# fcogidi/X3D-tf

Measured on AMD Instinct MI355X. Metric: clips/sec (fwd+bwd) X3D-M 16x224^2; depthwise HBM GB/s, higher is better.
Workload: dtype bf16

## Files before the change

### x3d-tf_amd/csrc/dw_mx.hip

```cpp
#include "dw_common.h"

#define MX_PITCH 48
#define MX_ROWS 18
#define MX_TILE (MX_PITCH * MX_ROWS)

struct DwMxFwdArgs {
  DwFwdArgs f;
  unsigned bytes;
};

template <typename T> struct MxOp;
template <> struct MxOp<bf16> {
  typedef bf16x8 x8;
  static __device__ __forceinline__ f32x4 mfma(x8 a, x8 b, f32x4 c) { return __builtin_amdgcn_mfma_f32_16x16x32_bf16(a, b, c, 0, 0, 0); }
};
template <> struct MxOp<f16> {
  typedef f16x8 x8;
  static __device__ __forceinline__ f32x4 mfma(x8 a, x8 b, f32x4 c) { return __builtin_amdgcn_mfma_f32_16x16x32_f16(a, b, c, 0, 0, 0); }
};

template <typename T, bool FLIP>
__device__ __forceinline__ void mx_weight_operands(const float* __restrict__ wc, int lane, typename MxOp<T>::x8 (&A)[6]) {
  const int w = lane & 15, g = lane >> 4;
  float wr[27];
#pragma unroll
  for (int k = 0; k < 27; k++) wr[k] = wc[k];
#pragma unroll
  for (int i = 0; i < 6; i++) {
    const int kt = i >> 1;
    float t3[3];
#pragma unroll
    for (int kw = 0; kw < 3; kw++) {
      float lo, hi;
      if (!FLIP) {
        lo = (i & 1) ? wr[kt * 9 + 6 + kw] : wr[kt * 9 + kw];
        hi = (i & 1) ? 0.f : wr[kt * 9 + 3 + kw];
      } else {
        lo = (i & 1) ? wr[(2 - kt) * 9 + 0 + (2 - kw)] : wr[(2 - kt) * 9 + 6 + (2 - kw)];
        hi = (i & 1) ? 0.f : wr[(2 - kt) * 9 + 3 + (2 - kw)];
      }
      t3[kw] = (g >> 1) ? hi : lo;
    }
    typename MxOp<T>::x8 a;
#pragma unroll
    for (int j = 0; j < 8; j++) {
      const int kw = 8 * (g & 1) + j - w + 1;
      const float v = kw == 0 ? t3[0] : (kw == 1 ? t3[1] : (kw == 2 ? t3[2] : 0.f));
      a[j] = (T)v;
    }
    A[i] = a;
  }
}

template <bool P7>
struct MxMap {
  int voffL, shift;
  int vst0, vst1, vst1e;
  unsigned mk0, mk1;
  int n;
  int planeB;
  __device__ __forceinline__ void build(int lane, int blk, int N, int C, int T, int H, int W, int& c) {
    const int h = lane & 15, s = lane >> 4;
    if constexpr (!P7) {
      c = __builtin_amdgcn_readfirstlane(blk % C);
      n = __builtin_amdgcn_readfirstlane(blk / C);
      const bool ok0 = h < H && 4 * s < W, ok1 = h < H && 4 * s + 2 < W;
      const long long e = (((long long)n * C + c) * T * H + h) * W + 4 * s;
      voffL = ok0 ? (int)(e * 2) : DW_OOB;
      shift = 0;
      vst0 = voffL;
      vst1 = ok1 ? (int)(e * 2) + 4 : DW_OOB;
      vst1e = DW_OOB;
      mk0 = ok0 ? 0xffffffffu : 0u;
      mk1 = ok1 ? 0xffffffffu : 0u;
      planeB = H * W * 2;
    } else {
      c = __builtin_amdgcn_readfirstlane(blk % C);
      const int n0 = __builtin_amdgcn_readfirstlane(blk / C) * 4;
      n = n0 + 2 * (h >> 3) + (s >> 1);
      const int r = h & 7, second = s & 1;
      const bool ok = r < 7 && n < N;
      const long long e = (((long long)n * C + c) * T * 7 + r) * 7 + 4 * second;
      voffL = ok ? (int)((e - second) * 2) : DW_OOB;
      shift = second;
      vst0 = ok ? (int)(e * 2) : DW_OOB;
      vst1 = (ok && !second) ? (int)(e * 2) + 4 : DW_OOB;
      vst1e = (ok && second) ? (int)(e * 2) + 4 : DW_OOB;
      mk0 = ok ? 0xffffffffu : 0u;
      mk1 = ok ? (second ? 0x0000ffffu : 0xffffffffu) : 0u;
      planeB = 49 * 2;
    }
  }
  __device__ __forceinline__ Raw aligned(const Raw& r) const {
    if constexpr (P7) {
      const unsigned long long v = (((unsigned long long)r.w[1] << 32) | r.w[0]) >> (16 * shift);
      Raw o; o.w[0] = (unsigned)v; o.w[1] = (unsigned)(v >> 32); o.w[2] = o.w[3] = 0u;
      return o;
    } else {
      return r;
    }
  }
  __device__ __forceinline__ void store(__amdgpu_buffer_rsrc_t rs, unsigned p0, unsigned p1, int soff) const {
    Raw o, o1;
    o.w[0] = p0; o1.w[0] = p1;
    raw_bstore<4>(o, rs, vst0, soff);
    raw_bstore<4>(o1, rs, vst1, soff);
    if constexpr (P7) raw_bstore<2>(o1, rs, vst1e, soff);
  }
};

template <typename T, int UN, int RB, int PD, bool EXACT, bool P7>
__global__ __launch_bounds__(64, 7) void dw3d_fwd_mx14_kernel(const DwMxFwdArgs pa) {
  static_assert(UN % RB == 0 && UN % PD == 0, "ring period RB, slots period PD");
  typedef typename MxOp<T>::x8 x8;
  __shared__ __attribute__((aligned(16))) unsigned char lds[RB * MX_TILE];
  const DwFwdArgs& a = pa.f;
  const DwGeom& g = a.g;
  const int lane = threadIdx.x;
  const int h = lane & 15, s = lane >> 4;
  int c;
  MxMap<P7> mp;
  mp.build(lane, blockIdx.x, g.N, g.C, g.T, g.H, g.W, c);

  for (int i = lane; i < RB * MX_TILE / 16; i += 64) ((uint4*)lds)[i] = make_uint4(0u, 0u, 0u, 0u);

  x8 A[6];
  mx_weight_operands<T, false>(a.w + c * 27, lane, A);
  float sc = 1.f, sh = 0.f;
  if (a.ss) { sc = a.ss[c * 2]; sh = a.ss[c * 2 + 1]; }
  const float lo = a.act == X3D_ACT_RELU ? 0.f : -__builtin_inff();

  const int planeB = mp.planeB;
  const __amdgpu_buffer_rsrc_t rsX = __builtin_amdgcn_make_buffer_rsrc((T*)a.x, 0, pa.bytes, 0x00020000);
  const __amdgpu_buffer_rsrc_t rsY = __builtin_amdgcn_make_buffer_rsrc((T*)a.y, 0, pa.bytes, 0x00020000);
  unsigned char* stg = lds + (h + 1) * MX_PITCH + s * 8;
  const unsigned char* rd01 = lds + (h + (s >> 1)) * MX_PITCH + (s & 1) * 16;
  const unsigned char* rd2 = lds + (h + 2) * MX_PITCH + (s & 1) * 16;

  Raw slot[PD];
  auto issue = [&](int t, Raw& r) { raw_bload<8>(r, rsX, mp.voffL, t < g.T ? t * planeB : DW_OOB); };
  const unsigned mk0 = mp.mk0, mk1 = mp.mk1;
  auto stage = [&](const Raw& r0, int q, bool plane_ok) {
    const Raw r = mp.aligned(r0);
    float v[4];
#pragma unroll
    for (int e = 0; e < 4; e++) v[e] = fmaxf(__builtin_fmaf(sc, raw_get<T>(r, e), sh), lo);
    const unsigned pm = plane_ok ? 0xffffffffu : 0u;
    *(uint2*)(stg + q * MX_TILE) = make_uint2(Dot2<T>::pk(v[0], v[1]) & (mk0 & pm), Dot2<T>::pk(v[2], v[3]) & (mk1 & pm));
  };
  float s1 = 0.f, s2 = 0.f;

  auto dummy_stores = [&]() { mp.store(rsY, 0u, 0u, DW_OOB); };
#pragma unroll
  for (int p = 0; p < PD; p++) { issue(p, slot[p]); dummy_stores(); }
  stage(slot[0], 1, true);
  issue(PD, slot[0]);
  dummy_stores();

  for (int t0 = 0; t0 < g.T; t0 += UN) {
#pragma unroll
    for (int d = 0; d < UN; d++) {
      const int t = t0 + d;
      if (!EXACT && t >= g.T) break;
      const int qm = d % RB, q0 = (d + 1) % RB, qp = (d + 2) % RB;
      stage(slot[(d + 1) % PD], qp, t + 1 < g.T);
      issue(t + 1 + PD, slot[(d + 1) % PD]);
      f32x4 acc = {0.f, 0.f, 0.f, 0.f}, acc2 = {0.f, 0.f, 0.f, 0.f};
      const int qs[3] = {qm, q0, qp};
#pragma unroll
      for (int kt = 0; kt < 3; kt++) {
        const x8 b01 = *(const x8*)(rd01 + qs[kt] * MX_TILE);
        const x8 b2 = *(const x8*)(rd2 + qs[kt] * MX_TILE);
        acc = MxOp<T>::mfma(A[2 * kt], b01, acc);
        acc2 = MxOp<T>::mfma(A[2 * kt + 1], b2, acc2);
      }
      acc += acc2;
      float o4[4];
#pragma unroll
      for (int e = 0; e < 4; e++) {
        const unsigned m = e < 2 ? mk0 : mk1;
        o4[e] = (m >> (16 * (e & 1)) & 1u) ? acc[e] : 0.f;
        s1 += o4[e];
        s2 += o4[e] * o4[e];
      }
      mp.store(rsY, Dot2<T>::pk(o4[0], o4[1]), Dot2<T>::pk(o4[2], o4[3]), t * planeB);
    }
  }
  if (a.stats || a.pool) {
    const float q1 = wave_sum(s1), q2 = wave_sum(s2);
    float qp[P7 ? 4 : 1];
    if constexpr (P7) {
#pragma unroll
      for (int k = 0; k < 4; k++) qp[k] = wave_sum((2 * (h >> 3) + (s >> 1)) == k ? s1 : 0.f);
    }
    if (lane == 0) {
      if (a.stats) {
        double* sp = stats_replica(a.stats, g.C, (unsigned)blockIdx.x);
        atomic_add_d(&sp[c * 2], (double)q1);
        atomic_add_d(&sp[c * 2 + 1], (double)q2);
      }
      if (a.pool) {
        if constexpr (P7) {
          const int n0 = (int)(blockIdx.x / g.C) * 4;
#pragma unroll
          for (int k = 0; k < 4; k++) if (n0 + k < g.N) atomic_add_d(&a.pool[(long long)(n0 + k) * g.C + c], (double)qp[k]);
        } else {
          atomic_add_d(&a.pool[(long long)mp.n * g.C + c], (double)q1);
        }
      }
    }
  }
}

static bool mx_plane_ok(const DwGeom& g, bool* p7) {
  *p7 = g.H == 7 && g.W == 7;
  return *p7 || (g.H >= 12 && g.H <= 14 && g.W >= 12 && g.W <= 14 && (g.W & 1) == 0);
}

bool dw_fwd_mx_launch(const DwFwdArgs& a, int dtype, int S, hipStream_t st) {
  const DwGeom& g = a.g;
  const int e = x3d_env_int("X3D_DW_MX", 1);
  bool p7;
  if (e == 0 || dtype == X3D_F32 || S != 1 || !mx_plane_ok(g, &p7) || a.bn.stats) return false;
  const long long bytes = (long long)g.N * g.C * g.T * g.H * g.W * 2;
  if (bytes >= (1ll << 30) || (long long)g.C * g.N >= (1ll << 31)) return false;
  if (((uintptr_t)a.x & 3) || ((uintptr_t)a.y & 3)) return false;
  const bool exact = g.T % 4 == 0;
  if (x3d_describe.out) {
    snprintf(x3d_describe.out, x3d_describe.cap, "dw3d_fwd_mx14_kernel<%s, %s, %d>", dtype == X3D_BF16 ? "bf16" : "f16",
             exact ? "4, 4, 4, 1" : "6, 3, 3, 0", (int)p7);
    return true;
  }
  DwMxFwdArgs pa;
  pa.f = a;
  pa.bytes = (unsigned)bytes;
  const dim3 grid((unsigned)(g.C * (p7 ? ceil_div(g.N, 4) : g.N)));
#define MX_FWD(TT, P7_)                                                                                             \
  do {                                                                                                              \
    if (exact) hipLaunchKernelGGL((dw3d_fwd_mx14_kernel<TT, 4, 4, 4, true, P7_>), grid, dim3(64), 0, st, pa);       \
    else hipLaunchKernelGGL((dw3d_fwd_mx14_kernel<TT, 6, 3, 3, false, P7_>), grid, dim3(64), 0, st, pa);            \
  } while (0)
  if (dtype == X3D_BF16) { if (p7) MX_FWD(bf16, true); else MX_FWD(bf16, false); }
  else { if (p7) MX_FWD(f16, true); else MX_FWD(f16, false); }
#undef MX_FWD
  return true;
}

#define MXA_PITCH 80
#define MXA_TILE (MXA_PITCH * MX_ROWS)

struct DwMxBwdArgs {
  DwBwdArgs b;
  unsigned bytes;
};

template <typename T, int UN, int RB, int PD, bool EXACT, bool P7>
__global__ __launch_bounds__(64, 3) void dw3d_bwd_mx14_kernel(const DwMxBwdArgs pa) {
  static_assert(UN % RB == 0 && UN % 2 == 0 && UN % PD == 0, "ring periods RB (dB planes), 2 (A planes) and PD (planes in flight)");
  typedef typename MxOp<T>::x8 x8;
  typedef __attribute__((ext_vector_type(4))) unsigned int u32x4_;
  __shared__ __attribute__((aligned(16))) unsigned char lds[RB * MX_TILE + 2 * MXA_TILE + 64];
  unsigned char* ldsA = lds + RB * MX_TILE;
  const DwBwdArgs& a = pa.b;
  const DwGeom& g = a.g;
  const int lane = threadIdx.x;
  const int h = lane & 15, s = lane >> 4;
  int c;
  MxMap<P7> mp;
  mp.build(lane, blockIdx.x, g.N, g.C, g.T, g.H, g.W, c);

  for (int i = lane; i < (RB * MX_TILE + 2 * MXA_TILE + 64) / 16; i += 64) ((uint4*)lds)[i] = make_uint4(0u, 0u, 0u, 0u);

  x8 Wt[6];
  mx_weight_operands<T, true>(a.w + c * 27, lane, Wt);
  const float sc = a.ss_a[c * 2], sh = a.ss_a[c * 2 + 1];
  float cA = 0.f, cB = 0.f, cC = 0.f;
  if (mp.n < g.N) {
    const float* cf = a.coef_nc + ((long long)mp.n * g.C + c) * 4;
    cA = cf[0]; cB = cf[1]; cC = cf[2];
  }
  const int planeB = mp.planeB;
  const __amdgpu_buffer_rsrc_t rsA = __builtin_amdgcn_make_buffer_rsrc((T*)a.araw, 0, pa.bytes, 0x00020000);
  const __amdgpu_buffer_rsrc_t rsD = __builtin_amdgcn_make_buffer_rsrc((T*)a.dv, 0, pa.bytes, 0x00020000);
  const __amdgpu_buffer_rsrc_t rsR = __builtin_amdgcn_make_buffer_rsrc((T*)a.braw, 0, pa.bytes, 0x00020000);
  const __amdgpu_buffer_rsrc_t rsG = __builtin_amdgcn_make_buffer_rsrc((T*)a.ga, 0, pa.bytes, 0x00020000);
  unsigned char* stgB = lds + (h + 1) * MX_PITCH + s * 8;
  const unsigned char* rd01 = lds + (h + (s >> 1)) * MX_PITCH + (s & 1) * 16;
  const unsigned char* rd2 = lds + (h + 2) * MX_PITCH + (s & 1) * 16;
  const bool lowk = s < 2;
  const unsigned char* rdM = lowk ? lds + (h + 1) * MX_PITCH + (s & 1) * 16 : lds + RB * MX_TILE + 2 * MXA_TILE;
  const int rdM_tile = lowk ? MX_TILE : 0;
  unsigned char* stgA = ldsA + (h + 1) * MXA_PITCH + 16 + s * 8;
  const unsigned char* rdN = ldsA + (h + 1) * MXA_PITCH + 16 + (s & 1) * 16;

  struct Slot { Raw A, D, R; };
  Slot slot[PD];
  auto issue = [&](int t, Slot& q) {
    const int soff = t < g.T ? t * planeB : DW_OOB;
    raw_bload<8>(q.A, rsA, mp.voffL, soff);
    raw_bload<8>(q.D, rsD, mp.voffL, soff);
    raw_bload<8>(q.R, rsR, mp.voffL, soff);
  };
  const unsigned mk0 = mp.mk0, mk1 = mp.mk1;
  auto stage = [&](const Slot& q, int qb, int qa, bool plane_ok) {
    const Raw rA = mp.aligned(q.A), rD = mp.aligned(q.D), rR = mp.aligned(q.R);
    float av[4], bv[4];
#pragma unroll
    for (int e = 0; e < 4; e++) {
      av[e] = fmaxf(__builtin_fmaf(sc, raw_get<T>(rA, e), sh), 0.f);
      bv[e] = __builtin_fmaf(cA, raw_get<T>(rD, e), __builtin_fmaf(cB, raw_get<T>(rR, e), cC));
    }
    const unsigned pm = plane_ok ? 0xffffffffu : 0u;
    const unsigned m0 = mk0 & pm, m1 = mk1 & pm;
    *(uint2*)(stgA + qa * MXA_TILE) = make_uint2(Dot2<T>::pk(av[0], av[1]) & m0, Dot2<T>::pk(av[2], av[3]) & m1);
    *(uint2*)(stgB + qb * MX_TILE) = make_uint2(Dot2<T>::pk(bv[0], bv[1]) & m0, Dot2<T>::pk(bv[2], bv[3]) & m1);
  };

  f32x4 Cw[9];
#pragma unroll
  for (int k = 0; k < 9; k++) Cw[k] = (f32x4){0.f, 0.f, 0.f, 0.f};
  float s1 = 0.f, s2 = 0.f;
  Raw own;

  auto dummy_stores = [&]() { mp.store(rsG, 0u, 0u, DW_OOB); };
#pragma unroll
  for (int p = 0; p < PD; p++) { issue(p, slot[p]); dummy_stores(); }
  stage(slot[0], 1, 0, true);
  own = mp.aligned(slot[0].A);
  issue(PD, slot[0]);
  dummy_stores();

  for (int t0 = 0; t0 < g.T; t0 += UN) {
#pragma unroll
    for (int d = 0; d < UN; d++) {
      const int t = t0 + d;
      if (!EXACT && t >= g.T) break;
      const int qs[3] = {d % RB, (d + 1) % RB, (d + 2) % RB};
      const int sl = (d + 1) % PD;
      stage(slot[sl], qs[2], (d + 1) & 1, t + 1 < g.T);
      const Raw own_next = mp.aligned(slot[sl].A);
      issue(t + 1 + PD, slot[sl]);
      f32x4 acc = {0.f, 0.f, 0.f, 0.f}, acc2 = {0.f, 0.f, 0.f, 0.f};
#pragma unroll
      for (int kt = 0; kt < 3; kt++) {
        const x8 b01 = *(const x8*)(rd01 + qs[kt] * MX_TILE);
        const x8 b2 = *(const x8*)(rd2 + qs[kt] * MX_TILE);
        acc = MxOp<T>::mfma(Wt[2 * kt], b01, acc);
        acc2 = MxOp<T>::mfma(Wt[2 * kt + 1], b2, acc2);
      }
      {
        const unsigned char* pn = rdN + (d & 1) * MXA_TILE;
        const u32x4_ mid = *(const u32x4_*)pn;
        const unsigned prv = *(const unsigned*)(pn - 4), nxt = *(const unsigned*)(pn + 16);
        const unsigned m01 = __builtin_amdgcn_alignbit(mid[1], mid[0], 16), m12 = __builtin_amdgcn_alignbit(mid[2], mid[1], 16),
                       m23 = __builtin_amdgcn_alignbit(mid[3], mid[2], 16);
        const u32x4_ lft = {__builtin_amdgcn_alignbit(mid[0], prv, 16), m01, m12, m23};
        const u32x4_ rgt = {m01, m12, m23, __builtin_amdgcn_alignbit(nxt, mid[3], 16)};
        const x8 n0 = __builtin_bit_cast(x8, lft), n1 = __builtin_bit_cast(x8, mid), n2 = __builtin_bit_cast(x8, rgt);
#pragma unroll
        for (int kt = 0; kt < 3; kt++) {
          const x8 m = *(const x8*)(rdM + qs[2 - kt] * rdM_tile);
          Cw[kt * 3 + 0] = MxOp<T>::mfma(m, n0, Cw[kt * 3 + 0]);
          Cw[kt * 3 + 1] = MxOp<T>::mfma(m, n1, Cw[kt * 3 + 1]);
          Cw[kt * 3 + 2] = MxOp<T>::mfma(m, n2, Cw[kt * 3 + 2]);
          }
      }
      acc += acc2;
      float o4[4];
#pragma unroll
      for (int e = 0; e < 4; e++) {
        const float av = raw_get<T>(own, e);
        o4[e] = (__builtin_fmaf(sc, av, sh) > 0.f && ((e < 2 ? mk0 : mk1) >> (16 * (e & 1)) & 1u)) ? acc[e] : 0.f;
        s1 += o4[e];
        s2 += o4[e] * av;
      }
      mp.store(rsG, Dot2<T>::pk(o4[0], o4[1]), Dot2<T>::pk(o4[2], o4[3]), t * planeB);
      own = own_next;
    }
  }

  float red[29];
#pragma unroll
  for (int kt = 0; kt < 3; kt++)
#pragma unroll
    for (int kw = 0; kw < 3; kw++) {
      float p[3] = {0.f, 0.f, 0.f};
#pragma unroll
      for (int r = 0; r < 4; r++) {
        const int kh = h - (4 * s + r) + 1;
        const float v = Cw[kt * 3 + kw][r];
        p[0] += kh == 0 ? v : 0.f;
        p[1] += kh == 1 ? v : 0.f;
        p[2] += kh == 2 ? v : 0.f;
      }
#pragma unroll
      for (int kh = 0; kh < 3; kh++) red[kt * 9 + kh * 3 + kw] = wave_sum_lane63(p[kh]);
    }
  red[27] = wave_sum_lane63(s1);
  red[28] = wave_sum_lane63(s2);
  dw_flush_sums29(red, lane, a.dw + c * 27, a.a_sums + c * 2);
}

bool dw_bwd_mx_launch(const DwBwdArgs& a, int dtype, int S, hipStream_t st) {
  const DwGeom& g = a.g;
  const int e = x3d_env_int("X3D_DW_MX", 1);
  bool p7;
  if (e == 0 || (dtype != X3D_BF16 && (dtype != X3D_F16 || x3d_env_int("X3D_DW_MX_F16", 1) == 0)) || S != 1 || !mx_plane_ok(g, &p7)) return false;
  if (p7 && e != 7) return false;
  const long long bytes = (long long)g.N * g.C * g.T * g.H * g.W * 2;
  if (bytes >= (1ll << 30) || (long long)g.C * g.N >= (1ll << 31)) return false;
  if (((uintptr_t)a.araw & 3) || ((uintptr_t)a.ga & 3) || ((uintptr_t)a.dv & 3) || ((uintptr_t)a.braw & 3)) return false;
  const bool exact = g.T % 4 == 0 && !(p7 && dtype != X3D_BF16);
  if (x3d_describe.out) {
    snprintf(x3d_describe.out, x3d_describe.cap, "dw3d_bwd_mx14_kernel<%s, %s, %d>", dtype == X3D_BF16 ? "bf16" : "f16", exact ? "4, 4, 2, 1" : "6, 3, 3, 0", (int)p7);
    return true;
  }
  DwMxBwdArgs pa;
  pa.b = a;
  pa.bytes = (unsigned)bytes;
  const dim3 grid((unsigned)(g.C * (p7 ? ceil_div(g.N, 4) : g.N)));
#define MX14_BWD(T_)                                                                                              \
  do {                                                                                                            \
    if (p7) {                                                                                                     \
      if (exact) hipLaunchKernelGGL((dw3d_bwd_mx14_kernel<T_, 4, 4, 2, true, true>), grid, dim3(64), 0, st, pa);    \
      else hipLaunchKernelGGL((dw3d_bwd_mx14_kernel<T_, 6, 3, 3, false, true>), grid, dim3(64), 0, st, pa);         \
    } else {                                                                                                      \
      if (exact) hipLaunchKernelGGL((dw3d_bwd_mx14_kernel<T_, 4, 4, 2, true, false>), grid, dim3(64), 0, st, pa);   \
      else hipLaunchKernelGGL((dw3d_bwd_mx14_kernel<T_, 6, 3, 3, false, false>), grid, dim3(64), 0, st, pa);        \
    }                                                                                                             \
  } while (0)
  if (dtype == X3D_BF16) MX14_BWD(bf16); else MX14_BWD(f16);
#undef MX14_BWD
  return true;
}


#define MXW_PITCH 112
#define MXW_TILE (MXW_PITCH * MX_ROWS)

struct DwMxwBwdArgs {
  DwBwdArgs b;
  unsigned bytes;
  int HT;
};

template <typename T, int UN, int RB, int PD, bool EXACT>
__global__ __launch_bounds__(64, 2) void dw3d_bwd_mxw_kernel(const DwMxwBwdArgs pa) {
  static_assert(UN % RB == 0 && UN % 2 == 0 && UN % PD == 0, "ring periods RB (dB planes), 2 (A planes) and PD (planes in flight)");
  typedef typename MxOp<T>::x8 x8;
  typedef __attribute__((ext_vector_type(4))) unsigned int u32x4_;
  __shared__ __attribute__((aligned(16))) unsigned char lds[(RB + 2) * MXW_TILE + 128];
  unsigned char* ldsA = lds + RB * MXW_TILE;
  const DwBwdArgs& a = pa.b;
  const DwGeom& g = a.g;
  const int lane = threadIdx.x;
  const int n16 = lane & 15, s = lane >> 4;
  const int ht = __builtin_amdgcn_readfirstlane(blockIdx.x % pa.HT);
  const int nc = __builtin_amdgcn_readfirstlane(blockIdx.x / pa.HT);
  const int c = nc % g.C, n = nc / g.C;
  const int H = g.H, W = g.W;
  const int r0 = ht * 14;

  for (int i = lane; i < ((RB + 2) * MXW_TILE + 128) / 16; i += 64) ((uint4*)lds)[i] = make_uint4(0u, 0u, 0u, 0u);

  x8 Wt[9];
  {
    const float* wc = a.w + c * 27;
#pragma unroll
    for (int i = 0; i < 9; i++) {
      const int kt = i / 3, kh = i % 3;
      const float* w3 = wc + (2 - kt) * 9 + (2 - kh) * 3;
      const float w0 = w3[2], w1 = w3[1], w2 = w3[0];
      x8 op;
#pragma unroll
      for (int j = 0; j < 8; j++) {
        const int kw = 8 * s + j - n16 - 7;
        op[j] = (T)(kw == 0 ? w0 : (kw == 1 ? w1 : (kw == 2 ? w2 : 0.f)));
      }
      Wt[i] = op;
    }
  }
  const float sc = a.ss_a[c * 2], sh = a.ss_a[c * 2 + 1];
  const float* cf = a.coef_nc + ((long long)n * g.C + c) * 4;
  const float cA = cf[0], cB = cf[1], cC = cf[2];

  const int planeB = H * W * 2;
  const __amdgpu_buffer_rsrc_t rsA = __builtin_amdgcn_make_buffer_rsrc((T*)a.araw, 0, pa.bytes, 0x00020000);
  const __amdgpu_buffer_rsrc_t rsD = __builtin_amdgcn_make_buffer_rsrc((T*)a.dv, 0, pa.bytes, 0x00020000);
  const __amdgpu_buffer_rsrc_t rsR = __builtin_amdgcn_make_buffer_rsrc((T*)a.braw, 0, pa.bytes, 0x00020000);
  const __amdgpu_buffer_rsrc_t rsG = __builtin_amdgcn_make_buffer_rsrc((T*)a.ga, 0, pa.bytes, 0x00020000);
  const int row = r0 - 1 + n16;
  const bool row_in = row >= 0 && row < H;
  const bool row_own = n16 >= 1 && n16 <= 14 && row < H;
  const long long base = ((long long)n * g.C + c) * g.T * H * W + (long long)row * W;
  int vld[2], vs0[2], vs1[2];
  unsigned mk0[2], mk1[2], eo0[2], eo1[2];
#pragma unroll
  for (int j = 0; j < 2; j++) {
    const int col = 16 * j + 4 * s;
    const bool c0 = col < W, c1 = col + 2 < W;
    vld[j] = (row_in && c0) ? (int)((base + col) * 2) : DW_OOB;
    mk0[j] = (row_in && c0) ? 0xffffffffu : 0u;
    mk1[j] = (row_in && c1) ? 0xffffffffu : 0u;
    eo0[j] = (row_own && c0) ? 1u : 0u;
    eo1[j] = (row_own && c1) ? 1u : 0u;
    vs0[j] = eo0[j] ? (int)((base + col) * 2) : DW_OOB;
    vs1[j] = eo1[j] ? (int)((base + col + 2) * 2) : DW_OOB;
  }
  unsigned char* stgB = lds + (n16 + 1) * MXW_PITCH + 16 + s * 8;
  unsigned char* stgA = ldsA + (n16 + 1) * MXW_PITCH + 16 + s * 8;
  const unsigned char* rdB = lds + n16 * MXW_PITCH + s * 16;
  const unsigned char* rdM = row_own ? lds + (n16 + 1) * MXW_PITCH + 16 + s * 16 : lds + (RB + 2) * MXW_TILE;
  const int rdM_tile = row_own ? MXW_TILE : 0;
  const unsigned char* rdN = ldsA + (n16 + 1) * MXW_PITCH + 16 + s * 16;

  struct Slot { Raw A[2], D[2], R[2]; };
  Slot slot[PD];
  auto issue = [&](int t, Slot& q) {
    const int soff = t < g.T ? t * planeB : DW_OOB;
#pragma unroll
    for (int j = 0; j < 2; j++) {
      raw_bload<8>(q.A[j], rsA, vld[j], soff);
      raw_bload<8>(q.D[j], rsD, vld[j], soff);
      raw_bload<8>(q.R[j], rsR, vld[j], soff);
    }
  };
  auto stage = [&](const Slot& q, int qb, int qa, bool plane_ok) {
    const unsigned pm = plane_ok ? 0xffffffffu : 0u;
#pragma unroll
    for (int j = 0; j < 2; j++) {
      float av[4], bv[4];
#pragma unroll
      for (int e = 0; e < 4; e++) {
        av[e] = fmaxf(__builtin_fmaf(sc, raw_get<T>(q.A[j], e), sh), 0.f);
        bv[e] = __builtin_fmaf(cA, raw_get<T>(q.D[j], e), __builtin_fmaf(cB, raw_get<T>(q.R[j], e), cC));
      }
      const unsigned m0 = mk0[j] & pm, m1 = mk1[j] & pm;
      *(uint2*)(stgA + qa * MXW_TILE + 32 * j) = make_uint2(Dot2<T>::pk(av[0], av[1]) & m0, Dot2<T>::pk(av[2], av[3]) & m1);
      *(uint2*)(stgB + qb * MXW_TILE + 32 * j) = make_uint2(Dot2<T>::pk(bv[0], bv[1]) & m0, Dot2<T>::pk(bv[2], bv[3]) & m1);
    }
  };
  auto store4 = [&](int j, unsigned p0, unsigned p1, int soff) {
    Raw o, o1;
    o.w[0] = p0; o1.w[0] = p1;
    raw_bstore<4>(o, rsG, vs0[j], soff);
    raw_bstore<4>(o1, rsG, vs1[j], soff);
  };
  auto dummy_stores = [&]() { store4(0, 0u, 0u, DW_OOB); store4(1, 0u, 0u, DW_OOB); };

  f32x4 Cw[9];
#pragma unroll
  for (int k = 0; k < 9; k++) Cw[k] = (f32x4){0.f, 0.f, 0.f, 0.f};
  float s1 = 0.f, s2 = 0.f;
  Raw own[2];

#pragma unroll
  for (int p = 0; p < PD; p++) { issue(p, slot[p]); dummy_stores(); }
  stage(slot[0], 1, 0, true);
  own[0] = slot[0].A[0]; own[1] = slot[0].A[1];
  issue(PD, slot[0]);
  dummy_stores();

  for (int t0 = 0; t0 < g.T; t0 += UN) {
#pragma unroll
    for (int d = 0; d < UN; d++) {
      const int t = t0 + d;
      if (!EXACT && t >= g.T) break;
      const int qs[3] = {d % RB, (d + 1) % RB, (d + 2) % RB};
      const int sl = (d + 1) % PD;
      stage(slot[sl], qs[2], (d + 1) & 1, t + 1 < g.T);
      const Raw on0 = slot[sl].A[0], on1 = slot[sl].A[1];
      issue(t + 1 + PD, slot[sl]);
      {
        const unsigned char* pn = rdN + (d & 1) * MXW_TILE;
        const u32x4_ mid = *(const u32x4_*)pn;
        const unsigned prv = *(const unsigned*)(pn - 4), nxt = *(const unsigned*)(pn + 16);
        const unsigned m01 = __builtin_amdgcn_alignbit(mid[1], mid[0], 16), m12 = __builtin_amdgcn_alignbit(mid[2], mid[1], 16),
                       m23 = __builtin_amdgcn_alignbit(mid[3], mid[2], 16);
        const u32x4_ lft = {__builtin_amdgcn_alignbit(mid[0], prv, 16), m01, m12, m23};
        const u32x4_ rgt = {m01, m12, m23, __builtin_amdgcn_alignbit(nxt, mid[3], 16)};
        const x8 n0 = __builtin_bit_cast(x8, lft), n1 = __builtin_bit_cast(x8, mid), n2 = __builtin_bit_cast(x8, rgt);
#pragma unroll
        for (int kt = 0; kt < 3; kt++) {
          const x8 m = *(const x8*)(rdM + qs[2 - kt] * rdM_tile);
          Cw[kt * 3 + 0] = MxOp<T>::mfma(m, n0, Cw[kt * 3 + 0]);
          Cw[kt * 3 + 1] = MxOp<T>::mfma(m, n1, Cw[kt * 3 + 1]);
          Cw[kt * 3 + 2] = MxOp<T>::mfma(m, n2, Cw[kt * 3 + 2]);
        }
      }
#pragma unroll
      for (int j = 0; j < 2; j++) {
        f32x4 acc = {0.f, 0.f, 0.f, 0.f}, acc2 = {0.f, 0.f, 0.f, 0.f}, acc3 = {0.f, 0.f, 0.f, 0.f};
#pragma unroll
        for (int kt = 0; kt < 3; kt++) {
          const unsigned char* pb = rdB + qs[kt] * MXW_TILE + 32 * j;
          acc = MxOp<T>::mfma(Wt[kt * 3 + 0], *(const x8*)(pb), acc);
          acc2 = MxOp<T>::mfma(Wt[kt * 3 + 1], *(const x8*)(pb + MXW_PITCH), acc2);
          acc3 = MxOp<T>::mfma(Wt[kt * 3 + 2], *(const x8*)(pb + 2 * MXW_PITCH), acc3);
        }
        acc += acc2 + acc3;
        float o4[4];
#pragma unroll
        for (int e = 0; e < 4; e++) {
          const float av = raw_get<T>(own[j], e);
          o4[e] = (__builtin_fmaf(sc, av, sh) > 0.f && (e < 2 ? eo0[j] : eo1[j])) ? acc[e] : 0.f;
          s1 += o4[e];
          s2 += o4[e] * av;
        }
        store4(j, Dot2<T>::pk(o4[0], o4[1]), Dot2<T>::pk(o4[2], o4[3]), t * planeB);
      }
      own[0] = on0; own[1] = on1;
    }
  }

  float red[29];
#pragma unroll
  for (int kt = 0; kt < 3; kt++)
#pragma unroll
    for (int kw = 0; kw < 3; kw++) {
      float p[3] = {0.f, 0.f, 0.f};
#pragma unroll
      for (int r = 0; r < 4; r++) {
        const int kh = n16 - (4 * s + r) + 1;
        const float v = Cw[kt * 3 + kw][r];
        p[0] += kh == 0 ? v : 0.f;
        p[1] += kh == 1 ? v : 0.f;
        p[2] += kh == 2 ? v : 0.f;
      }
#pragma unroll
      for (int kh = 0; kh < 3; kh++) red[kt * 9 + kh * 3 + kw] = wave_sum_lane63(p[kh]);
    }
  red[27] = wave_sum_lane63(s1);
  red[28] = wave_sum_lane63(s2);
  dw_flush_sums29(red, lane, a.dw + c * 27, a.a_sums + c * 2);
}

bool dw_bwd_mxw_launch(const DwBwdArgs& a, int dtype, int S, hipStream_t st) {
  const DwGeom& g = a.g;
  const int e = x3d_env_int("X3D_DW_MXW", 1);
  if (e == 0 || (dtype != X3D_BF16 && (dtype != X3D_F16 || x3d_env_int("X3D_DW_MX_F16", 1) == 0)) || S != 1 || (g.W & 1) || g.W < 26 || g.W > 30 || g.H < 12 ||
      (g.H % 14 != 0 && g.H % 14 < 10)) return false;
  const long long bytes = (long long)g.N * g.C * g.T * g.H * g.W * 2;
  const int HT = ceil_div(g.H, 14);
  if (bytes >= (1ll << 30) || (long long)g.C * g.N * HT >= (1ll << 31)) return false;
  if (((uintptr_t)a.araw & 7) || ((uintptr_t)a.ga & 3) || ((uintptr_t)a.dv & 7) || ((uintptr_t)a.braw & 7)) return false;
  const bool exact = g.T % 4 == 0 && dtype == X3D_BF16;
  if (x3d_describe.out) {
    snprintf(x3d_describe.out, x3d_describe.cap, "dw3d_bwd_mxw_kernel<%s, %s>", dtype == X3D_BF16 ? "bf16" : "f16", exact ? "4, 4, 2, 1" : "6, 3, 3, 0");
    return true;
  }
  DwMxwBwdArgs pa;
  pa.b = a;
  pa.bytes = (unsigned)bytes;
  pa.HT = HT;
  const dim3 grid((unsigned)((long long)g.C * g.N * HT));
  if (dtype == X3D_BF16) {
    if (exact) hipLaunchKernelGGL((dw3d_bwd_mxw_kernel<bf16, 4, 4, 2, true>), grid, dim3(64), 0, st, pa);
    else hipLaunchKernelGGL((dw3d_bwd_mxw_kernel<bf16, 6, 3, 3, false>), grid, dim3(64), 0, st, pa);
  } else {
    if (exact) hipLaunchKernelGGL((dw3d_bwd_mxw_kernel<f16, 4, 4, 2, true>), grid, dim3(64), 0, st, pa);
    else hipLaunchKernelGGL((dw3d_bwd_mxw_kernel<f16, 6, 3, 3, false>), grid, dim3(64), 0, st, pa);
  }
  return true;
}
```

Measured before the change: 3198.

## Process multiple batch samples per wave in depthwise weight-grad kernel with cross-sample streaming

The backward depthwise MFMA kernel now assigns several batch samples of the same channel and row tile to one wave, instead of one sample per wave. Weight-gradient accumulators stay in registers across samples, so each wave does one reduction and flush for all of them. In the exact path the load pipeline runs straight into the next sample, and that sample's first plane is staged early, which avoids draining and refilling the prefetch at sample boundaries. The number of samples per wave is cut back when the grid would otherwise be too small to fill the device. This adds per-sample coefficient selection and extra double-precision atomics for the activation sums, and it reduces parallelism.

```diff
diff --git a/x3d-tf_amd/csrc/dw_mx.hip b/x3d-tf_amd/csrc/dw_mx.hip
--- a/x3d-tf_amd/csrc/dw_mx.hip
+++ b/x3d-tf_amd/csrc/dw_mx.hip
@@ -442,11 +442,32 @@
   DwBwdArgs b;
   unsigned bytes;
   int HT;
+  int k;
 };
+
+#define MXW_SAMPLES 2
+#define MX_SAMPLES_MAX 4
+static int mx_samples_per_wave(int k, long long waves, int waves_per_simd) {
+  const int e = x3d_env_int("X3D_DW_MX_K", 0);
+  if (e > 0) return e < MX_SAMPLES_MAX ? e : MX_SAMPLES_MAX;
+  const long long slots = (long long)x3d_device_cus() * 4 * waves_per_simd;
+  while (k > 1 && waves / k < 2 * slots) k >>= 1;
+  return k;
+}
+
+__device__ __forceinline__ float mx_pick(const float (&kc)[MX_SAMPLES_MAX][3], int j, int e) {
+  float v = kc[MX_SAMPLES_MAX - 1][e];
+#pragma unroll
+  for (int q = MX_SAMPLES_MAX - 2; q >= 0; q--) v = j == q ? kc[q][e] : v;
+  return v;
+}
 
 template <typename T, int UN, int RB, int PD, bool EXACT>
 __global__ __launch_bounds__(64, 2) void dw3d_bwd_mxw_kernel(const DwMxwBwdArgs pa) {
   static_assert(UN % RB == 0 && UN % 2 == 0 && UN % PD == 0, "ring periods RB (dB planes), 2 (A planes) and PD (planes in flight)");
+  constexpr bool STREAM = EXACT;
+  static_assert(!STREAM || (RB == 4 && UN == 4 && PD < 4), "the stream parks the next sample's plane 0 in the ring's fourth slot; "
+                                                           "it looks PD planes into the next sample (T >= 4)");
   typedef typename MxOp<T>::x8 x8;
   typedef __attribute__((ext_vector_type(4))) unsigned int u32x4_;
   __shared__ __attribute__((aligned(16))) unsigned char lds[(RB + 2) * MXW_TILE + 128];
@@ -456,8 +477,10 @@
   const int lane = threadIdx.x;
   const int n16 = lane & 15, s = lane >> 4;
   const int ht = __builtin_amdgcn_readfirstlane(blockIdx.x % pa.HT);
-  const int nc = __builtin_amdgcn_readfirstlane(blockIdx.x / pa.HT);
-  const int c = nc % g.C, n = nc / g.C;
+  const int c = __builtin_amdgcn_readfirstlane(blockIdx.x / pa.HT);
+  const int n = (int)(blockIdx.y + blockIdx.z * 65535u) * pa.k;
+  if (n >= g.N) return;
+  const int ns = min(pa.k, g.N - n);
   const int H = g.H, W = g.W;
   const int r0 = ht * 14;
 
@@ -482,9 +505,22 @@
   }
   const float sc = a.ss_a[c * 2], sh = a.ss_a[c * 2 + 1];
   const float* cf = a.coef_nc + ((long long)n * g.C + c) * 4;
-  const float cA = cf[0], cB = cf[1], cC = cf[2];
+  float cA = cf[0], cB = cf[1], cC = cf[2];
+  float kc[MX_SAMPLES_MAX][3];
+#pragma unroll
+  for (int j = 0; j < MX_SAMPLES_MAX; j++) {
+    const float* cn = a.coef_nc + ((long long)(n + min(j, ns - 1)) * g.C + c) * 4;
+    kc[j][0] = cn[0]; kc[j][1] = cn[1]; kc[j][2] = cn[2];
+  }
+  float nA, nB, nC;
+  auto next_coef = [&](int i) { nA = mx_pick(kc, i + 1, 0); nB = mx_pick(kc, i + 1, 1); nC = mx_pick(kc, i + 1, 2); };
+  next_coef(0);
 
   const int planeB = H * W * 2;
+  const int sampB = g.C * g.T * planeB;
+  int sb = 0;
+  bool more = STREAM && ns > 1;
+  int pastB = more ? sampB - g.T * planeB : DW_OOB, pastM = more ? planeB : 0;
   const __amdgpu_buffer_rsrc_t rsA = __builtin_amdgcn_make_buffer_rsrc((T*)a.araw, 0, pa.bytes, 0x00020000);
   const __amdgpu_buffer_rsrc_t rsD = __builtin_amdgcn_make_buffer_rsrc((T*)a.dv, 0, pa.bytes, 0x00020000);
   const __amdgpu_buffer_rsrc_t rsR = __builtin_amdgcn_make_buffer_rsrc((T*)a.braw, 0, pa.bytes, 0x00020000);
@@ -517,7 +553,8 @@
   struct Slot { Raw A[2], D[2], R[2]; };
   Slot slot[PD];
   auto issue = [&](int t, Slot& q) {
-    const int soff = t < g.T ? t * planeB : DW_OOB;
+    const bool in = t < g.T;
+    const int soff = (in ? sb : pastB) + t * (in ? planeB : pastM);
 #pragma unroll
     for (int j = 0; j < 2; j++) {
       raw_bload<8>(q.A[j], rsA, vld[j], soff);
@@ -525,7 +562,7 @@
       raw_bload<8>(q.R[j], rsR, vld[j], soff);
     }
   };
-  auto stage = [&](const Slot& q, int qb, int qa, bool plane_ok) {
+  auto stage = [&](const Slot& q, int qb, int qa, bool plane_ok, bool NEXT0 = false, int qn = 0) {
     const unsigned pm = plane_ok ? 0xffffffffu : 0u;
 #pragma unroll
     for (int j = 0; j < 2; j++) {
@@ -536,8 +573,15 @@
         bv[e] = __builtin_fmaf(cA, raw_get<T>(q.D[j], e), __builtin_fmaf(cB, raw_get<T>(q.R[j], e), cC));
       }
       const unsigned m0 = mk0[j] & pm, m1 = mk1[j] & pm;
-      *(uint2*)(stgA + qa * MXW_TILE + 32 * j) = make_uint2(Dot2<T>::pk(av[0], av[1]) & m0, Dot2<T>::pk(av[2], av[3]) & m1);
+      const unsigned a0 = NEXT0 ? mk0[j] : m0, a1 = NEXT0 ? mk1[j] : m1;
+      *(uint2*)(stgA + qa * MXW_TILE + 32 * j) = make_uint2(Dot2<T>::pk(av[0], av[1]) & a0, Dot2<T>::pk(av[2], av[3]) & a1);
       *(uint2*)(stgB + qb * MXW_TILE + 32 * j) = make_uint2(Dot2<T>::pk(bv[0], bv[1]) & m0, Dot2<T>::pk(bv[2], bv[3]) & m1);
+      if (NEXT0) {
+        float nv[4];
+#pragma unroll
+        for (int e = 0; e < 4; e++) nv[e] = __builtin_fmaf(nA, raw_get<T>(q.D[j], e), __builtin_fmaf(nB, raw_get<T>(q.R[j], e), nC));
+        *(uint2*)(stgB + qn * MXW_TILE + 32 * j) = make_uint2(Dot2<T>::pk(nv[0], nv[1]) & mk0[j], Dot2<T>::pk(nv[2], nv[3]) & mk1[j]);
+      }
     }
   };
   auto store4 = [&](int j, unsigned p0, unsigned p1, int soff) {
@@ -552,15 +596,20 @@
 #pragma unroll
   for (int k = 0; k < 9; k++) Cw[k] = (f32x4){0.f, 0.f, 0.f, 0.f};
   float s1 = 0.f, s2 = 0.f;
+  double d1 = 0.0, d2 = 0.0;
   Raw own[2];
 
-#pragma unroll
-  for (int p = 0; p < PD; p++) { issue(p, slot[p]); dummy_stores(); }
-  stage(slot[0], 1, 0, true);
-  own[0] = slot[0].A[0]; own[1] = slot[0].A[1];
-  issue(PD, slot[0]);
-  dummy_stores();
-
+  auto prologue = [&]() {
+#pragma unroll
+    for (int p = 0; p < PD; p++) { issue(p, slot[p]); dummy_stores(); }
+    stage(slot[0], 1, 0, true);
+    own[0] = slot[0].A[0]; own[1] = slot[0].A[1];
+    issue(PD, slot[0]);
+    dummy_stores();
+  };
+  prologue();
+
+  for (int i = 0;;) {
   for (int t0 = 0; t0 < g.T; t0 += UN) {
 #pragma unroll
     for (int d = 0; d < UN; d++) {
@@ -568,7 +617,7 @@
       if (!EXACT && t >= g.T) break;
       const int qs[3] = {d % RB, (d + 1) % RB, (d + 2) % RB};
       const int sl = (d + 1) % PD;
-      stage(slot[sl], qs[2], (d + 1) & 1, t + 1 < g.T);
+      stage(slot[sl], qs[2], (d + 1) & 1, t + 1 < g.T, STREAM && d == UN - 1, (d + 3) % RB);
       const Raw on0 = slot[sl].A[0], on1 = slot[sl].A[1];
       issue(t + 1 + PD, slot[sl]);
       {
@@ -607,10 +656,26 @@
           s1 += o4[e];
           s2 += o4[e] * av;
         }
-        store4(j, Dot2<T>::pk(o4[0], o4[1]), Dot2<T>::pk(o4[2], o4[3]), t * planeB);
+        store4(j, Dot2<T>::pk(o4[0], o4[1]), Dot2<T>::pk(o4[2], o4[3]), sb + t * planeB);
       }
       own[0] = on0; own[1] = on1;
     }
+  }
+    if (++i >= ns) break;
+    d1 += (double)wave_sum_lane63(s1);
+    d2 += (double)wave_sum_lane63(s2);
+    s1 = 0.f; s2 = 0.f;
+#pragma unroll
+    for (int j = 0; j < 2; j++) {
+      if constexpr (STREAM) *(uint2*)(stgB + MXW_TILE + 32 * j) = *(const uint2*)(stgB + 2 * MXW_TILE + 32 * j);
+      *(uint2*)(stgB + 32 * j) = make_uint2(0u, 0u);
+    }
+    sb += sampB;
+    cA = nA; cB = nB; cC = nC;
+    more = STREAM && i + 1 < ns;
+    pastB = more ? sb + sampB - g.T * planeB : DW_OOB; pastM = more ? planeB : 0;
+    next_coef(i);
+    if constexpr (!STREAM) prologue();
   }
 
   float red[29];
@@ -633,6 +698,10 @@
   red[27] = wave_sum_lane63(s1);
   red[28] = wave_sum_lane63(s2);
   dw_flush_sums29(red, lane, a.dw + c * 27, a.a_sums + c * 2);
+  if (ns > 1 && lane == 63) {
+    atomicAdd(&a.a_sums[c * 2], d1);
+    atomicAdd(&a.a_sums[c * 2 + 1], d2);
+  }
 }
 
 bool dw_bwd_mxw_launch(const DwBwdArgs& a, int dtype, int S, hipStream_t st) {
@@ -653,7 +722,9 @@
   pa.b = a;
   pa.bytes = (unsigned)bytes;
   pa.HT = HT;
-  const dim3 grid((unsigned)((long long)g.C * g.N * HT));
+  pa.k = mx_samples_per_wave(MXW_SAMPLES, (long long)g.C * g.N * HT, 2);
+  const int groups = ceil_div(g.N, pa.k);
+  const dim3 grid((unsigned)(g.C * HT), (unsigned)(groups < 65535 ? groups : 65535), (unsigned)ceil_div(groups, 65535));
   if (dtype == X3D_BF16) {
     if (exact) hipLaunchKernelGGL((dw3d_bwd_mxw_kernel<bf16, 4, 4, 2, true>), grid, dim3(64), 0, st, pa);
     else hipLaunchKernelGGL((dw3d_bwd_mxw_kernel<bf16, 6, 3, 3, false>), grid, dim3(64), 0, st, pa);
```

Result: no change. 3215, median of 6 (+0.5%).
